# lbroseus/TALC

Hardware: AMD Instinct MI355X
Metric: corrected long-read bases/sec (whole node); k-mer-probe HBM GB/s (higher is better)
Workload: dtype u8

## Files before the change

talc_amd/csrc/pure_capi.cpp:

```cpp
#include <algorithm>
#include <cstdint>
#include <vector>

#include "talc_pure.h"
#include "talc_wfa.h"

using namespace talc;

extern "C" {

int pure_is_expected_by_model(double alpha, uint32_t nextc, uint32_t cc, int classe_unexpected) {
  return is_expected_by_model(alpha, nextc, cc, classe_unexpected != 0) ? 1 : 0;
}
int pure_is_expected_by_last_node(double alpha, uint32_t nextc, uint32_t cc) {
  return is_expected_by_last_node(alpha, nextc, cc) ? 1 : 0;
}
int pure_tag_next_nodes(double alpha, double err, uint32_t minc, const uint32_t* cnt4, const uint32_t* jc4, uint32_t count,
                        int complex, int32_t* tags4, double* dist4) {
  int t[4];
  double d[4];
  int n = tag_next_nodes(alpha, err, minc, cnt4, jc4, count, complex != 0, t, d);
  for (int i = 0; i < 4; ++i) { tags4[i] = t[i]; dist4[i] = d[i]; }
  return n;
}
// ... 16 lines not shown
void pure_gnu_heapsort_pairs(int32_t* keys, int32_t* payloads, int n) {
  std::vector<KP> v(n);
  for (int i = 0; i < n; ++i) v[i] = KP{keys[i], payloads[i]};
  gs_heapsort(v.data(), 0, n, KPLess());
  for (int i = 0; i < n; ++i) { keys[i] = v[i].key; payloads[i] = v[i].payload; }
}
void pure_std_heapsort_pairs(int32_t* keys, int32_t* payloads, int n) {
  std::vector<KP> v(n);
  for (int i = 0; i < n; ++i) v[i] = KP{keys[i], payloads[i]};
  std::partial_sort(v.begin(), v.end(), v.end(), KPLess());
  for (int i = 0; i < n; ++i) { keys[i] = v[i].key; payloads[i] = v[i].payload; }
}

int pure_gardening(uint32_t maxb, int n, const double* scores, const double* dists, uint32_t* kept, int32_t* isComplex) {
  std::vector<ValIdx> wv(n + 1);
  std::vector<Rank4> r1(n + 1), r2(n + 1);
  bool cx = false;
  int nk = gardening(maxb, n, scores, dists, wv.data(), r1.data(), r2.data(), kept, &cx);
  *isComplex = cx ? 1 : 0;
  return nk;
}

void pure_sort_anchors(double cc, uint32_t* pos, uint32_t* count, int n) {
  std::vector<AnchorRec> a(n);
  for (int i = 0; i < n; ++i) a[i] = AnchorRec{0, 0, pos[i], count[i]};
  gnu_sort(a.data(), n, LessAnchor{cc});
  for (int i = 0; i < n; ++i) { pos[i] = a[i].pos; count[i] = a[i].count; }
}

void pure_wfa_xdrop(const uint8_t* q, int qlen, const uint8_t* d, int dlen, int x, int32_t* out4) {
  const WfaResult r = wfa_xdrop_scalar(q, qlen, d, dlen, x);
  out4[0] = r.moved; out4[1] = r.extCols; out4[2] = r.extRows; out4[3] = r.score;
}
}
```

talc_amd/csrc/talc_kernels_search.h:

```cpp
#pragma once
#include "talc_common.h"
#include "talc_kernels_probe.h"
#include "talc_pure.h"
#include "talc_wave.h"

namespace talc {

#define TCAP 288
#define NBUF (2 * TCAP)
#ifndef LDS_DP_CAP
#define LDS_DP_CAP 320
#endif
#ifndef HOT
#define HOT 8
#endif
#ifndef AIMS_LDS
#define AIMS_LDS 16
#endif

enum : uint32_t {
  OVF_ANCHORS = 1, OVF_FULLPATHS = 2, OVF_FULLPOOL = 4, OVF_TRAILS = 8, OVF_SEQ = 16, OVF_OUT = 32, OVF_WEAKPOOL = 64,
  OVF_REGIONS = 128, OVF_DP = 256
};

// ... 504 lines not shown
struct TrailSet {
  uint64_t* kmer; uint64_t* nmask; double* dist; uint32_t* cnt; int32_t* score; uint32_t* fail; int32_t* lanc;
  int32_t* ranc; uint32_t* buf;
};
TALC_D TrailSet make_set(uint8_t* meta) {
  TrailSet s;
  s.kmer = (uint64_t*)(meta + TrailSetLayout::kmer); s.nmask = (uint64_t*)(meta + TrailSetLayout::nmask);
  s.dist = (double*)(meta + TrailSetLayout::dist); s.cnt = (uint32_t*)(meta + TrailSetLayout::cnt);
  s.score = (int32_t*)(meta + TrailSetLayout::score); s.fail = (uint32_t*)(meta + TrailSetLayout::fail);
  s.lanc = (int32_t*)(meta + TrailSetLayout::lanc); s.ranc = (int32_t*)(meta + TrailSetLayout::ranc);
  s.buf = (uint32_t*)(meta + TrailSetLayout::buf);
  return s;
}

struct TrailRec { uint64_t kmer, nmask; double dist; uint32_t cnt; int32_t score; uint32_t fail; int32_t lanc, ranc; uint32_t buf; };

#define LSYNC() do { __builtin_amdgcn_fence(__ATOMIC_ACQ_REL, "wavefront"); __builtin_amdgcn_wave_barrier(); } while (0)

__shared__ TrailRec g_hot[2 * HOT];
__shared__ uint64_t g_aimK[AIMS_LDS], g_aimN[AIMS_LDS];
__shared__ uint32_t g_aimPos[AIMS_LDS];
#define BLOOM_WORDS 128
__shared__ unsigned long long g_bloom[BLOOM_WORDS];
__shared__ __attribute__((aligned(16))) int g_dp[3 * LDS_DP_CAP];

struct EdgeCand {
  bool have; double score; double dist; double idscore; uint32_t len; uint32_t lanc, ranc;
};

enum { PF_PROBE = 0, PF_CHILD, PF_AIMS, PF_CYCLE, PF_FFWD, PF_SCOREBR, PF_GARDEN, PF_EVALFULL, PF_XDROP, PF_EXTNW,
       PF_EDGEMISC, PF_ANCHORS, PF_ASSEMBLE, PF_STEPB, PF_STEPE, PF_SRCHB, PF_SRCHE, PF_PROLOG, PF_INITTR, PF_TOTAL, PF_NCALLS, PF_NSTEPS,
       PF_FFLOAD, PF_FFREC, PF_FFFLUSH, PF_FFENTRY, PF_NRECS, PF_RD0, PF_RD1, PF_RD2, PF_RD3, PF_RD4, PF_RD5, PF_RDMAX,
       PF_XSTAGE, PF_XLEV, PF_XSEL, PF_REFB, PF_RESULT, PF_CYQ, PF_CYX, PF_CYHIT, PF_CYFILL,
       PF_SB11, PF_SB12, PF_SB21, PF_SB10, PF_SBOTHER, PF_SEGEN, PF_XCALLS, PF_XNLEV, PF_FSFORK, PF_FSDEAD, PF_FSFILT, PF_FSLIM, PF_FK1, PF_FK2, PF_FKBAIL, PF_FORK, PF_ANCCALLS, PF_ANCITER, PF_TPUB, PF_TOWN, PF_TSTOLEN, PF_TWAIT, PF_TRUN, PF_EA0, PF_EA1, PF_EA2, PF_EA3, PF_EA4, PF_EASUM3, PF_EASUM4, PF_RANCH, PF_RANCHMAX, PF_RBR, PF_RBRMAX, PF_N };
#define TALC_PF_NAMES {"probe", "child", "aims", "cycle", "ffwd", "scorebr", "garden", "evalfull", "xdrop", "extnw", "edgemisc", \
                       "anchors", "assemble", "stepb*", "stepe*", "srchb*", "srche*", "prolog", "inittr", "total", "#ffcalls", "#ffsteps", \
                       "ff.load", "ff.record", "ff.flush", "ff.entry", "#ffrecords", "#reads<0.25ms", "#reads<1ms", "#reads<4ms", \
                       "#reads<16ms", "#reads<64ms", "#reads>=64ms", "maxread(10ns)", "x.stage", "x.levels", "x.select", "b.ref", "b.result", \
                       "#cyc.query", "#cyc.exact", "#cyc.found", "cyc.fill%sum", \
                       "#stepb 1->1", "#stepb 1->2", "#stepb 2->1", "#stepb 1->0", "#stepb other", "#stepe generic", "#xdrop calls", "#xdrop levels", \
                       "#ffstop fork", "#ffstop deadend", "#ffstop filter", "#ffstop limit/other", "#forkstep 1 child", "#forkstep fork+deadend", "#forkstep bailed", "forkstep", "#anchor lists", "#anchor level tests", \
                       "#edges published", "#anchors by owner", "#anchors by others", "t.owner waits", "t.run by others", \
                       "#edge anchors<1ms", "#edge anchors<4ms", "#edge anchors<16ms", "#edge anchors<64ms", "#edge anchors>=64ms", "ticks anchors 16-64ms", "ticks anchors>=64ms", "(per read) anchors", "(per read) longest anchor", "(per read) bridge attempts", "(per read) longest bridge attempt"}

struct Wv {
  DevParams P; TableView T; SearchLimits C;
  const uint8_t* read; uint32_t L, n; const uint2* cov; double lambda;
  TrailSet G[2];
  int ia;
  uint8_t* seqPool;
  uint32_t nBuf;
  unsigned long long freeMask[NBUF / 64];
  uint8_t *ref, *fullPool, *edgeLong, *edgeShort, *edgeTmp, *weak;
  AnchorRec *ancL, *ancR; uint32_t* ancPos;
  FullMeta* fullMeta;
  int *dpG;
  double* gScores; double* gDists; ValIdx* gVal; Rank4* gRank; uint32_t* gKept;
  uint32_t *regS, *regE, *wOff, *wLen;
  int location, dirRight;
  uint32_t Ls, Le, Rs, Re;
  uint32_t weakLen;
  bool complexRegion;
  bool ffPopped;
  int nAncL, nAncR;
  uint32_t refLen;
  int nFull; uint32_t fullUsed;
  EdgeCand best2[2];
  int nEdges;
  unsigned long long cells, steps;
  uint32_t overflow;
  const TraceBuf* tracep;
  bool tracing, traceSteps;
  unsigned long long* wideBloom;
  int* rowPool;
  uint32_t searchNo;
  uint32_t rowStride, rowAvail;
// ... 552 lines not shown
      wave_xdrop<int*, false>(q, qlen, d, dlen, 0, -1, -1, xdrop, buf, extCols, extRows, ncells);
  }
  X.cells += ncells;
  return ((unsigned long long)(uint32_t)uni(extRows) << 32) | (uint32_t)uni(extCols);
}

struct SeedExt { int lenRefExt, lenHistExt, posOnRef, score; bool stop; int extRef, extCand; bool fallback; };

template <int MODE, bool LEAF = false>
TALC_D SeedExt seed_and_extension_body(const uint8_t* ref, int refLen, const uint8_t* cand, int candLen, int xdrop,
                                       bool withScore, uint32_t keepKey = 0) {
  PROF_DECL;
  refLen = uni(refLen); candLen = uni(candLen); xdrop = uni(xdrop); ref = uni_ptr(ref); cand = uni_ptr(cand);
  const int K = (int)X.P.K;
  const int S = X.dirRight ? K - 1 : K;
  SeedExt r;
  r.stop = false; r.score = 0; r.fallback = false;
  const bool state = !(refLen < candLen);
  const uint8_t* seq1 = state ? ref : cand; const int len1 = state ? refLen : candLen;
  const uint8_t* seq2 = state ? cand : ref; const int len2 = state ? candLen : refLen;
  int extCols = 0, extRows = 0, extScore = 0, rc = 0;
  unsigned long long ncells = 0;
  const int qlen = len2 - S, dlen = len1 - S;
  if (qlen > 0 && dlen > 0) {
    PROF_BEGIN();
#ifdef TALC_PROF
    if (lane_id() == 0) g_prof[PF_XCALLS] += 1;
#endif
    constexpr int STAGE = 3 * LDS_DP_CAP * 4;
    uint8_t TALC_AS3* stage = (uint8_t TALC_AS3*)g_dp;
    const int ndiagonals = min(max(xdrop, 0), qlen) + min(max(xdrop, 0), dlen) + 1;
    if (MODE == 2) {
      int* mem = X.dpG + 2ull * X.C.dpCap + 256;
      WfaPhase ph{-1, 31, mem, mem + 512};
      rc = wave_xdrop_wfa<1>(seq2 + S, qlen, seq1 + S, dlen, xdrop, stage, STAGE, extCols, extRows, extScore, ncells, &ph);
      if (rc == 2) {
        ph.fromLevel = 31; ph.toLevel = 63;
        rc = wave_xdrop_wfa<2>(seq2 + S, qlen, seq1 + S, dlen, xdrop, stage, STAGE, extCols, extRows, extScore, ncells, &ph);
        if (rc == 2) {
          ph.fromLevel = 63; ph.toLevel = 127;
          rc = wave_xdrop_wfa<4>(seq2 + S, qlen, seq1 + S, dlen, xdrop, stage, STAGE, extCols, extRows, extScore, ncells, &ph);
          if (rc == 2) {
            ph.fromLevel = 127; ph.toLevel = (ndiagonals <= 511) ? -1 : 255;
            rc = wave_xdrop_wfa<8>(seq2 + S, qlen, seq1 + S, dlen, xdrop, stage, STAGE, extCols, extRows, extScore, ncells, &ph);
            if (rc == 2) {
              ph.fromLevel = 255; ph.toLevel = -1;
              rc = wave_xdrop_wfa<16>(seq2 + S, qlen, seq1 + S, dlen, xdrop, stage, STAGE, extCols, extRows, extScore, ncells, &ph);
            }
          }
        }
      }
    }
    else if (MODE == 0 && ndiagonals <= 63) rc = wave_xdrop_wfa<1>(seq2 + S, qlen, seq1 + S, dlen, xdrop, stage, STAGE, extCols, extRows, extScore, ncells, nullptr, state ? keepKey : 0u);
    else if (MODE == 1 && ndiagonals <= 255) {
      int* mem = X.dpG + 2ull * X.C.dpCap + 256;
      WfaPhase ph{-1, 31, mem, mem + 512};
      rc = wave_xdrop_wfa<1>(seq2 + S, qlen, seq1 + S, dlen, xdrop, stage, STAGE, extCols, extRows, extScore, ncells, &ph, state ? keepKey : 0u);
      if (rc == 2) {
        ph.fromLevel = 31; ph.toLevel = (ndiagonals <= 127) ? -1 : 63;
        rc = wave_xdrop_wfa<2>(seq2 + S, qlen, seq1 + S, dlen, xdrop, stage, STAGE, extCols, extRows, extScore, ncells, &ph);
        if (rc == 2) {
          ph.fromLevel = 63; ph.toLevel = -1;
          rc = wave_xdrop_wfa<4>(seq2 + S, qlen, seq1 + S, dlen, xdrop, stage, STAGE, extCols, extRows, extScore, ncells, &ph);
        }
      }
    }
    else rc = -1;
    if (LEAF && rc < 0) { r.fallback = true; return r; }
    if (rc < 0) {
      rc = -1;
      const unsigned long long packed = xdrop_sweep(seq2 + S, qlen, seq1 + S, dlen, xdrop);
      extCols = (int)(uint32_t)packed; extRows = (int)(uint32_t)(packed >> 32);
    }
    PROF_END(PF_XDROP);
    X.cells += ncells;
  }
  const int ext1 = extRows, ext2 = extCols;
  r.extRef = state ? ext1 : ext2;
  r.extCand = state ? ext2 : ext1;
  r.lenRefExt = S + r.extRef;
  r.lenHistExt = S + r.extCand;
  r.posOnRef = X.dirRight ? (S + r.extRef) : (refLen - K - r.extRef);
  if (max(r.lenRefExt, r.lenHistExt) >= K) {
    if (withScore) {
      bool sameAnchor = LEAF && rc == 1;
      if (LEAF && !sameAnchor) { r.fallback = true; return r; }
      if (!LEAF && rc == 1) {
        const int l = lane_id();
        sameAnchor = ballot64(l < S && ((gcu8)ref)[l < S ? l : 0] != ((gcu8)cand)[l < S ? l : 0]) == 0ull;
      }
// ... 1927 lines not shown
  X.ia = 0;
  X.seqPool = slot + C.o_seqPool;
  X.refBuf = slot + C.o_ref; X.ref = X.refBuf; X.ancL = (AnchorRec*)(slot + C.o_ancL); X.ancR = (AnchorRec*)(slot + C.o_ancR);
  X.ancPos = (uint32_t*)(slot + C.o_ancPos);
  X.fullMeta = (FullMeta*)(slot + C.o_fullMeta); X.fullPool = slot + C.o_fullPoolB;
  X.edgeLong = slot + C.o_edgeLong; X.edgeShort = slot + C.o_edgeShort; X.edgeTmp = slot + C.o_edgeTmp;
  X.dpG = (int*)(slot + C.o_dp);
  X.wideBloom = (unsigned long long*)(slot + C.o_wideBloom); X.wideMask = 0;
  X.rowPool = (int*)(slot + C.o_rowPool); X.rowStride = 0; X.rowAvail = 0;
  X.launchStamp = launchStamp;
  if (E.boxes != nullptr && E.autoSwitch != nullptr && *E.autoSwitch == 0u) E.boxes = nullptr;
  X.boxes = E.boxes; X.avail = E.avail; X.qwords = queue; X.boxSeqCap = E.seqCap; X.boxBytes = (uint32_t)edge_box_bytes(E.seqCap);
  X.nSlots = gridDim.x; X.mySlot = blockIdx.x; X.nWork = n_work; X.taskMinWeak = E.minWeak; X.nanSeen = 0u; X.taskTest = E.test;
  X.taskHeavy = E.heavy; X.heavyUpTo = (E.heavyRounds >= 0xFFFFu) ? 0xFFFFFFFFu : E.heavyRounds * gridDim.x;
  X.qi = 0; X.holding = 0u; X.stealSeq = 0u; X.moreCells = 0; X.moreSteps = 0;
  const uint32_t lingerMod = max(E.lingerMod, 1u);
  X.searchNo = 16u;
  {
    uint8_t* g = slot + C.o_gard;
    X.gScores = (double*)g; g += 8ull * (TCAP + 64);
    X.gDists = (double*)g; g += 8ull * (TCAP + 64);
    X.gVal = (ValIdx*)g; g += 16ull * (TCAP + 64);
    X.gRank = (Rank4*)g; g += 32ull * (TCAP + 64);
    X.gKept = (uint32_t*)g;
  }
  X.regS = (uint32_t*)(slot + C.o_regS); X.regE = (uint32_t*)(slot + C.o_regE); X.regH = (uint32_t*)(slot + C.o_regH);
  X.wOff = (uint32_t*)(slot + C.o_wOff); X.wLen = (uint32_t*)(slot + C.o_wLen);
  X.weak = slot + C.o_weak;
  if (l == 0) *(TraceBuf*)(slot + C.o_trace) = trace;
  X.tracep = (const TraceBuf*)(slot + C.o_trace);
  unsigned long long totCells = 0, totSteps = 0;
  PROF_DECL2;
#ifdef TALC_PROF
  if (l == 0) { for (int i = 0; i < PF_N; ++i) g_prof[i] = 0; for (int i = 0; i < 4; ++i) g_wprof[i] = 0; }
  const unsigned long long _pf_k0 = __builtin_amdgcn_s_memtime();
  const unsigned long long _pf_r0 = __builtin_amdgcn_s_memrealtime();
  unsigned long long _pf_rd0 = 0, _pf_lastStart = 0, _pf_loopEnd = 0, _pf_idle = 0;
  uint32_t _pf_prevQi = 0, _pf_prevR = 0;
#endif

  while (true) {
    WSYNC();
#ifdef TALC_PROF
    if (l == 0 && _pf_rd0) {
      const unsigned long long dt = __builtin_amdgcn_s_memrealtime() - _pf_rd0;
      const int bk = dt < 25000ull ? 0 : dt < 100000ull ? 1 : dt < 400000ull ? 2 : dt < 1600000ull ? 3 : dt < 6400000ull ? 4 : 5;
      g_prof[PF_RD0 + bk] += 1;
      if (dt > g_prof[PF_RDMAX]) g_prof[PF_RDMAX] = (uint32_t)dt;
      state[_pf_prevR].pfTicks = (uint32_t)dt;
      _pf_lastStart = _pf_rd0; _pf_rd0 = 0;
    }
#endif
    if (X.boxes != nullptr) edge_between_reads();
    if (l == 0) s_next = atomicAdd(queue, 1u);
    WSYNC();
    const uint32_t qi = s_next;
    if (qi >= n_work) break;
    X.qi = qi;
#ifdef TALC_PROF
    _pf_rd0 = __builtin_amdgcn_s_memrealtime();
#endif
    PROF_BEGIN2();
    const uint32_t r = order[qi];
#ifdef TALC_PROF
    if (l == 0) state[r].pfStart = (uint32_t)_pf_rd0;
#endif
#ifdef TALC_PROF
// ... 134 lines not shown
        if (X.wLen[i] != 0xFFFFFFFFu) { copy_bytes(out + pos, X.weak + X.wOff[i], X.wLen[i], false); pos += X.wLen[i]; }
        else if (X.regS[i + 1] > e + K) { const uint32_t wl = X.regS[i + 1] - (e + K); copy_bytes(out + pos, X.read + e + K, wl, false); pos += wl; }
      }
    }
    if (tailPresent) {
      if (tailCorr) { copy_bytes(out + pos, X.weak + tailOff, tailCLen, false); pos += tailCLen; }
      else { copy_bytes(out + pos, X.read + (L - tailLen), tailLen, false); pos += tailLen; }
    }
    {
      unsigned long long part = 0;
      for (uint32_t i = l; i < R; i += 64) part += (unsigned long long)X.regE[i] - X.regS[i] + 1;
      const uint32_t span = (uint32_t)wave_sum_u64(part);
      if (l == 0) { state[r].outLen = pos; state[r].inSpan = span; }
    }
    PROF_END2(PF_ASSEMBLE);
  }
#ifdef TALC_PROF
  _pf_loopEnd = __builtin_amdgcn_s_memrealtime();
  if (l == 0) atomicMin((unsigned long long*)&counters[124], _pf_loopEnd);
#endif
  if (X.boxes != nullptr && blockIdx.x % lingerMod == 0u) {
#ifdef TALC_PROF
    _pf_idle =
#endif
    edge_linger(n_work);
  }
  totCells += X.moreCells; totSteps += X.moreSteps;
  if (l == 0) {
    if (totSteps) atomicAdd((unsigned long long*)&counters[0], totSteps);
    if (totCells) atomicAdd((unsigned long long*)&counters[1], totCells);
#ifdef TALC_PROF
    g_prof[PF_TOTAL] = (uint32_t)(__builtin_amdgcn_s_memtime() - _pf_k0);
    g_prof[PF_XSTAGE] = g_wprof[0]; g_prof[PF_XLEV] = g_wprof[1]; g_prof[PF_XSEL] = g_wprof[2]; g_prof[PF_XNLEV] = g_wprof[3];
    {
      const unsigned long long r1 = __builtin_amdgcn_s_memrealtime();
      atomicAdd((unsigned long long*)&counters[125], r1 - _pf_r0 - _pf_idle);
      atomicMin((unsigned long long*)&counters[126], _pf_r0);
      atomicMax((unsigned long long*)&counters[127], r1);
      if (_pf_rd0) state[_pf_prevR].pfTicks = (uint32_t)(r1 - _pf_rd0);
      if (blockIdx.x < 8192u) {
        counters[128 + 2 * blockIdx.x] = ((unsigned long long)_pf_prevQi << 32) | _pf_prevR;
        counters[129 + 2 * blockIdx.x] = ((_pf_lastStart & 0xFFFFFFFFull) << 32) | (_pf_loopEnd & 0xFFFFFFFFull);
      }
      static_assert(2 + PF_N <= 124, "the profile categories run into the utilisation counters");
    }
    for (int i = 0; i < PF_N; ++i) {
      if (i == PF_RDMAX) atomicMax((unsigned long long*)&counters[2 + i], (unsigned long long)g_prof[i]);
      else atomicAdd((unsigned long long*)&counters[2 + i], (unsigned long long)g_prof[i]);
    }
#endif
  }
}

TALC_D uint32_t order_bucket(const ReadState& st, uint32_t gapScale) {
  if (st.status != TALC_READ_CORRECTED || st.overflow) return 1023u;
  const unsigned long long key = (unsigned long long)st.costEst + (((unsigned long long)st.costGap * (gapScale - 256u)) >> 8);
  const uint32_t c = (uint32_t)min(key, 0xFFFFFFFFull) | 1u;
  const int e = 31 - __builtin_clz(c);
  const uint32_t m = (e >= 5) ? ((c >> (e - 5)) & 31u) : ((c << (5 - e)) & 31u);
  return 1022u - min(1022u, (uint32_t)e * 32u + m);
}
__global__ void __launch_bounds__(64) k_order_scale(uint32_t* __restrict__ batchStats) {
  const int l = lane_id();
  const unsigned long long fork = wave_sum_u64(batchStats[2 * l]), solid = wave_sum_u64(batchStats[2 * l + 1]);
  uint32_t scale = 256u;
  if (solid > 0) {
// ... 160 lines not shown
```

talc_amd/csrc/talc_wave.h:

```cpp
#pragma once
#include <limits.h>

#include "talc_common.h"

namespace talc {

#define WSYNC() __syncthreads()

TALC_D int lane_id() { return (int)__builtin_amdgcn_mbcnt_hi(~0u, __builtin_amdgcn_mbcnt_lo(~0u, 0u)); }
TALC_D int lane_id_here() { int l = lane_id(); asm volatile("" : "+v"(l)); return l; }
#define TALC_WAVE_REDUCE(v, OP, IDENT)                                                                   \
  do {                                                                                                   \
    v = OP(v, __builtin_amdgcn_update_dpp(IDENT, v, 0x111, 0xF, 0xF, false));                            \
    v = OP(v, __builtin_amdgcn_update_dpp(IDENT, v, 0x112, 0xF, 0xF, false));                            \
    v = OP(v, __builtin_amdgcn_update_dpp(IDENT, v, 0x114, 0xF, 0xF, false));                            \
    v = OP(v, __builtin_amdgcn_update_dpp(IDENT, v, 0x118, 0xF, 0xF, false));                            \
    v = OP(v, __builtin_amdgcn_update_dpp(IDENT, v, 0x142, 0xA, 0xF, false));                            \
    v = OP(v, __builtin_amdgcn_update_dpp(IDENT, v, 0x143, 0xC, 0xF, false));                            \
  } while (0)
TALC_D int wave_max_i32(int v) {
  TALC_WAVE_REDUCE(v, max, INT_MIN);
  return __builtin_amdgcn_readlane(v, 63);
}
TALC_D int talc_or_i32(int a, int b) { return a | b; }
// ... 516 lines not shown
    int mn, mx;
    minmaxS(A, false, mn, mx);
    const int lo = max(1 + mn, A + 3 - rows), hi = min(2 + mx, cols);
    early = lo >= hi;
  }
  if (!early) return firstMax(A);
  int maxColA = 1;
  if (A >= 2) {
    int mn1, mx1, mn2, mx2;
    minmaxS(A - 1, true, mn1, mx1);
    minmaxS(A - 2, false, mn2, mx2);
    const int cm = max(mx1, mx2);
    maxColA = (cm == INT_MIN) ? cols : min(2 + cm, cols);
  }
  const int c2 = maxColA - 1;
  if (kept(A, c2)) { take(A, c2); return 1; }
  if (A >= 2 && kept(A, c2 - 1)) { take(A, c2 - 1); return 1; }
  return firstMax(A - 1);
}

TALC_D void stage_copy(uint8_t TALC_AS3* dst, gcu8 src, int n) {
  const int l = lane_id_here();
  typedef uint64_t __attribute__((aligned(1))) u64u;
  const int nw = n >> 3;
  for (int w = l; w < nw; w += 64) ((uint64_t TALC_AS3*)dst)[w] = *(const u64u TALC_AS1*)(src + 8 * w);
  const int t = (nw << 3) + l;
  if (t < n) dst[t] = src[t];
}

struct WfaPhase {
  int fromLevel;
  int toLevel;
  int* memF; int* memE;
};

#ifdef TALC_PROF
__shared__ uint32_t g_wprof[4];
#define WPROF_T() __builtin_amdgcn_s_memtime()
#define WPROF_ADD(i, t0) (g_wprof[i] += (uint32_t)(__builtin_amdgcn_s_memtime() - (t0)))
#else
#define WPROF_T() 0ull
#define WPROF_ADD(i, t0) ((void)(t0))
#endif

struct WfaKeep { uint32_t owner; int level; int qlenAt; int pad_; uint16_t F[64]; uint8_t E[64]; };
__shared__ WfaKeep g_keep;

template <int NR>
TALC_D int wave_xdrop_wfa(const uint8_t* __restrict__ querySeg_, int qlen, const uint8_t* __restrict__ dbSeg_, int dlen, int x,
                          uint8_t TALC_AS3* stage, int stageCap, int& extCols, int& extRows, int& extScore,
                          unsigned long long& cells, const WfaPhase* ph = nullptr, uint32_t keepKey_ = 0) {
  gcu8 querySeg = (gcu8)uni_ptr(querySeg_); gcu8 dbSeg = (gcu8)uni_ptr(dbSeg_);
  const int l = lane_id();
  qlen = uni(qlen); dlen = uni(dlen); x = uni(x);
  extCols = extRows = extScore = 0;
  if (qlen <= 0 || dlen <= 0) return 0;
  const int NEG = -(1 << 29);
  const int X = min(max(x, 0), 1 << 20);
  const int fromLevel = ph ? ph->fromLevel : -1, toLevel = ph ? ph->toLevel : -1;
  const int Xm = (toLevel >= 0) ? min(X, toLevel) : X;
  const int kmin = -min(Xm, dlen), kmax = min(Xm, qlen);
  const int nd = kmax - kmin + 1;
  if (nd > 64 * NR - 1) return -1;
  const int qS = min(qlen, dlen + X), dS = min(dlen, qlen + X);
  const int qpad = (qS + 16) & ~7;
  if (qpad + dS + 16 > stageCap) return -1;
  const unsigned long long _t0 = WPROF_T();
  if (fromLevel < 0) {
    stage_copy(stage, querySeg, qS);
    stage_copy(stage + qpad, dbSeg, dS);
    if (l == 0) { stage[qS] = 0xF0; stage[qpad + dS] = 0xF1; }
  }
  WSYNC();
  WPROF_ADD(0, _t0);
  const unsigned long long _t1 = WPROF_T();
  const int bmax = x >= 2 ? x - 1 : (x == 1 ? 1 : 0);
  const int corner = qlen + dlen;
  int F[NR], E[NR], amax[NR], forb[NR];
#pragma unroll
  for (int s = 0; s < NR; ++s) {
    const int j = 64 * s + l, k = kmin + j, ak = k < 0 ? -k : k;
    amax[s] = (j < nd) ? min(2 * qlen - k, 2 * dlen + k) : NEG;
    forb[s] = (ak == bmax + 1) ? ak : -1;
    F[s] = NEG; E[s] = 0;
  }
  auto extend = [&](int (&a)[NR], bool (&act)[NR]) { wfa_extend<NR>(stage, qpad, kmin, a, act); };
  bool cornerHit = false;
  int cornerE = 0;
  int eStart = 1;
  const uint32_t keepKey = (NR == 1 && fromLevel < 0) ? (uint32_t)uni((int)keepKey_) : 0u;
  bool tracking = keepKey != 0u;
  const int kOfLane = kmin + l;
  const int aq = 2 * qlen - kOfLane;
  bool resumed = false;
  if (NR == 1 && keepKey != 0u) {
    const int lv = uni(g_keep.level), qat = uni(g_keep.qlenAt);
// ... 11 lines not shown
    if (level >= 1 && level <= 31) {
      if (l < nd) { g_keep.F[(kOfLane + 32) & 63] = (uint16_t)(F[0] >= 0 ? F[0] : 0xFFFF); g_keep.E[(kOfLane + 32) & 63] = (uint8_t)E[0]; }
      if (l == 0) { g_keep.owner = keepKey; g_keep.level = level; g_keep.qlenAt = qlen; }
    }
  };
  if (resumed) {
  } else
  if (fromLevel >= 0) {
#pragma unroll
    for (int s = 0; s < NR; ++s) {
      const int j = 64 * s + l, k = kmin + j, ak = k < 0 ? -k : k;
      const bool in = (j < nd) & (ak <= fromLevel);
      F[s] = in ? ph->memF[in ? k + 256 : 256] : NEG;
      E[s] = in ? ph->memE[in ? k + 256 : 256] : 0;
    }
    eStart = fromLevel + 1;
  } else {
    int a0[NR]; bool act0[NR];
    const int j0 = -kmin;
#pragma unroll
    for (int s = 0; s < NR; ++s) { a0[s] = 0; act0[s] = (64 * s + l == j0) && x >= 0; }
    extend(a0, act0);
#pragma unroll
    for (int s = 0; s < NR; ++s) if (64 * s + l == j0) F[s] = a0[s];
    unsigned long long hit = 0;
#pragma unroll
    for (int s = 0; s < NR; ++s) hit |= ballot64(F[s] == corner);
    cornerHit = hit != 0ull;
    if (tracking && ballot64(F[0] == aq) != 0ull) tracking = false;
  }
  const int eEnd = (toLevel >= 0) ? min(x, toLevel) : x;
  unsigned long long work = 0;
  const int kc = qlen - dlen;
  const bool cornerInBand = (kc >= kmin) & (kc <= kmax);
  int eLast = eStart - 1;
  for (int e = eStart; e <= eEnd && !cornerHit; ++e) {
    if (NR == 1 && tracking && e == x) { keep_level(e - 1); tracking = false; }
    const bool forbLevel = (e == bmax + 1);
    int rotR[NR], rotL[NR];
#pragma unroll
    for (int s = 0; s < NR; ++s) { rotR[s] = lane_ror1(F[s]); rotL[s] = lane_rol1(F[s]); }
    const int sLo = max(0, -e - kmin) >> 6, sHi = min(nd - 1, e - kmin) >> 6;
    int b[NR]; bool act[NR];
#pragma unroll
    for (int s = 0; s < NR; ++s) {
      b[s] = NEG; act[s] = false;
      if (NR == 1 || (s >= sLo && s <= sHi)) {
        const int fl = (NR > 1 && l == 0) ? rotR[(s + NR - 1) % NR] : rotR[s];
        const int fr = (NR > 1 && l == 63) ? rotL[(s + 1) % NR] : rotL[s];
        int v2 = fl + 1; v2 = (v2 <= amax[s]) ? v2 : NEG;
        int v3 = fr + 1; v3 = (v3 <= amax[s]) ? v3 : NEG;
        int v = max(max(v2, v3), min(F[s] + 2, amax[s]));
        if (forbLevel) v = (v == forb[s]) ? NEG : v;
        b[s] = v;
        act[s] = (v > F[s]) & (v >= 0);
      }
    }
    bool moved[NR];
#pragma unroll
    for (int s = 0; s < NR; ++s) moved[s] = act[s];
    extend(b, act);
    if (NR == 1 && tracking && ballot64(b[0] == aq) != 0ull) {
      keep_level(e - 1);
      tracking = false;
    }
    unsigned long long hit = 0;
#pragma unroll
    for (int s = 0; s < NR; ++s) {
      if (moved[s]) { F[s] = b[s]; E[s] = e; }
      if (cornerInBand) hit |= ballot64(F[s] == corner);
    }
    if (hit != 0ull) { cornerHit = true; cornerE = e; }
    eLast = e;
  }
  if (NR == 1 && tracking && !cornerHit && eLast < x) keep_level(eLast);
  if (eLast >= eStart) {
    const int eh = min(eLast, (nd - 1) / 2);
    const int lo = max(eh, eStart - 1);
    if (eh >= eStart) work += (unsigned long long)((eh - eStart + 1) * (eh + eStart + 1));
    if (eLast > lo) work += (unsigned long long)((eLast - lo) * nd);
  }
  cells += work;
  WPROF_ADD(1, _t1);
#ifdef TALC_PROF
  if (eLast >= eStart) g_wprof[3] += (uint32_t)(eLast - eStart + 1);
#endif
  const unsigned long long _t2 = WPROF_T();
  if (cornerHit) { extCols = qlen; extRows = dlen; extScore = -cornerE; return 1; }
  if (toLevel >= 0 && toLevel < x) {
#pragma unroll
    for (int s = 0; s < NR; ++s) {
      const int j = 64 * s + l, k = kmin + j, ak = k < 0 ? -k : k;
      if ((j < nd) & (ak <= toLevel)) { ph->memF[k + 256] = F[s]; ph->memE[k + 256] = E[s]; }
    }
    WSYNC();
    return 2;
  }
  const int rsel = wfa_select<NR>(F, E, kmin, kmax, qlen, dlen, extCols, extRows, extScore);
  WPROF_ADD(2, _t2);
  return rsel;
}

template <int NR>
TALC_D int wave_xdrop_wfa_multi(const uint8_t* __restrict__ querySeg_, int qlen, const uint8_t* __restrict__ dbSeg_, int dlen, int xHi,
                                uint8_t TALC_AS3* stage, int stageCap, int* resCols, int* resRows, int* resScore,
                                unsigned long long& cells) {
  gcu8 querySeg = (gcu8)uni_ptr(querySeg_); gcu8 dbSeg = (gcu8)uni_ptr(dbSeg_);
  const int l = lane_id();
  qlen = uni(qlen); dlen = uni(dlen); xHi = uni(xHi);
  if (qlen <= 0 || dlen <= 0 || xHi < 0) return -1;
  const int NEG = -(1 << 29);
  const int X = min(xHi, 1 << 20);
  const int kmin = -min(X, dlen), kmax = min(X, qlen);
  const int nd = kmax - kmin + 1;
  if (nd > 64 * NR - 1) return -1;
  const int qS = min(qlen, dlen + X), dS = min(dlen, qlen + X);
  const int qpad = (qS + 16) & ~7;
  if (qpad + dS + 16 > stageCap) return -1;
  stage_copy(stage, querySeg, qS);
  stage_copy(stage + qpad, dbSeg, dS);
  if (l == 0) { stage[qS] = 0xF0; stage[qpad + dS] = 0xF1; }
  WSYNC();
  const int corner = qlen + dlen;
  int F[NR], E[NR], amax[NR], ak[NR];
#pragma unroll
  for (int s = 0; s < NR; ++s) {
    const int j = 64 * s + l, k = kmin + j;
    ak[s] = k < 0 ? -k : k;
    amax[s] = (j < nd) ? min(2 * qlen - k, 2 * dlen + k) : NEG;
    F[s] = NEG; E[s] = 0;
  }
// ... 315 lines not shown
```

talc_amd/csrc/talc_wfa.h:

```cpp
#pragma once
#include <climits>
#include <cstdint>
#include <vector>

namespace talc {

struct WfaResult { int moved; int extCols; int extRows; int score; };

inline WfaResult wfa_xdrop_scalar(const uint8_t* q, int qlen, const uint8_t* d, int dlen, int x) {
  WfaResult res = {0, 0, 0, 0};
  if (qlen == 0 || dlen == 0) return res;
  const int NEG = -(1 << 29);
  const int bmax = x >= 2 ? x - 1 : (x == 1 ? 1 : 0);
  const int X = x < 0 ? 0 : x;
  const int kmin = -(X < dlen ? X : dlen), kmax = (X < qlen ? X : qlen);
  const int nd = kmax - kmin + 1;
  std::vector<int> F(nd + 2, NEG), G(nd + 2, NEG), E(nd + 2, 0), amin(nd + 2), amax(nd + 2);
  auto idx = [&](int k) { return k - kmin + 1; };
  for (int k = kmin; k <= kmax; ++k) {
    const int ak = k < 0 ? -k : k;
    amin[idx(k)] = ak + (ak > bmax ? 2 : 0);
    const int a1 = 2 * qlen - k, a2 = 2 * dlen + k;
    amax[idx(k)] = a1 < a2 ? a1 : a2;
  }
  auto extend = [&](int a, int k) {
    int c = (a + k) / 2, r = (a - k) / 2;
    while (c < qlen && r < dlen && q[c] == d[r]) { ++c; ++r; }
    return c + r;
  };
  const int corner = qlen + dlen, kc = qlen - dlen;
  F[idx(0)] = x >= 0 ? extend(0, 0) : 0;
  bool cornerHit = (kc >= kmin && kc <= kmax && F[idx(kc)] == corner);
  int cornerE = 0;
  for (int e = 1; e <= x && !cornerHit; ++e) {
    for (int k = kmin; k <= kmax; ++k) {
      const int i = idx(k);
      const int fm = F[i], fl = F[i - 1], fr = F[i + 1];
      int best = NEG;
      const int v[3] = {fm + 2, fl + 1, fr + 1};
      for (int t = 0; t < 3; ++t)
        if (v[t] >= amin[i] && v[t] <= amax[i] && v[t] > best) best = v[t];
      int nv = fm;
      if (best > fm) { nv = extend(best, k); E[i] = e; }
      G[i] = nv;
    }
    F.swap(G);
    if (kc >= kmin && kc <= kmax && F[idx(kc)] == corner) { cornerHit = true; cornerE = e; }
  }
  if (cornerHit) { res.moved = 1; res.extCols = qlen; res.extRows = dlen; res.score = -cornerE; return res; }
  int A = 0;
  for (int k = kmin; k <= kmax; ++k) if (F[idx(k)] > A) A = F[idx(k)];
  const int cols = qlen + 1, rows = dlen + 1;
  auto minmaxS = [&](int a, bool dropTopBorder, int& mn, int& mx) {
    mn = INT_MAX; mx = INT_MIN;
    if (a < 0) return;
    for (int k = kmin; k <= kmax; ++k) {
      if (((k - a) & 1) || F[idx(k)] < a) continue;
      const int c = (a + k) / 2;
      if (dropTopBorder && c == a) continue;
      if (c < mn) mn = c;
      if (c > mx) mx = c;
    }
  };
  auto kept = [&](int a, int c) {
    const int k = 2 * c - a;
    return c >= 0 && a - c >= 0 && k >= kmin && k <= kmax && F[idx(k)] >= a;
  };
  auto firstMax = [&](int a) {
    int bestE = INT_MAX, bestK = 0;
    for (int k = kmin; k <= kmax; ++k) {
      if (((k - a) & 1) || F[idx(k)] != a) continue;
      if (E[idx(k)] < bestE) { bestE = E[idx(k)]; bestK = k; }
    }
    if (bestE == INT_MAX) return;
    res.moved = 1; res.extCols = (a + bestK) / 2; res.extRows = (a - bestK) / 2; res.score = -bestE;
  };
  bool early = false;
  if (A + 1 >= 2) {
    int mn, mx; minmaxS(A, false, mn, mx);
    const int a = A + 1;
// ... 27 lines not shown
```

Before: 4.654 billion.

## Run X-drop WFA past level 31 in a sliding one-wave diagonal window

Adds a windowed mode to the single-register WFA kernel. Once three adjacent diagonals have reached the query end, diagonals above them are treated as dead, so the 64-lane band is shifted downward by bpermute instead of escalating to the multi-register (NR=2/4) phases. This targets the cost of wider-band phases for long X-drop extensions. It adds a ballot and permute per shifted level, a bail-out path when the window cannot shift, a scalar reference that implements the same pruning, and an exhaustive equivalence checker. Correctness depends on the pruning rule exactly matching the full-band result.

Result: faster. 4.716 billion, median of 6 (+1.3%).

```diff
diff --git a/talc_amd/csrc/pure_capi.cpp b/talc_amd/csrc/pure_capi.cpp
--- a/talc_amd/csrc/pure_capi.cpp
+++ b/talc_amd/csrc/pure_capi.cpp
@@ -72,4 +72,30 @@
   const WfaResult r = wfa_xdrop_scalar(q, qlen, d, dlen, x);
   out4[0] = r.moved; out4[1] = r.extCols; out4[2] = r.extRows; out4[3] = r.score;
 }
+void pure_wfa_xdrop_full(const uint8_t* q, int qlen, const uint8_t* d, int dlen, int x, int32_t* out4) {
+  const WfaResult r = wfa_xdrop_scalar(q, qlen, d, dlen, x, false);
+  out4[0] = r.moved; out4[1] = r.extCols; out4[2] = r.extRows; out4[3] = r.score;
 }
+int pure_wfa_window_exhaustive(int maxQ, int maxD, int xLo, int xHi, int64_t* runs, int32_t* first5) {
+  int bad = 0;
+  int64_t n = 0;
+  uint8_t q[32], d[32];
+  for (int ql = 1; ql <= maxQ; ++ql)
+    for (uint32_t qb = 0; qb < (1u << ql); ++qb)
+      for (int dl = 1; dl <= maxD; ++dl)
+        for (uint32_t db = 0; db < (1u << dl); ++db) {
+          for (int i = 0; i < ql; ++i) q[i] = (uint8_t)((qb >> i) & 1u);
+          for (int i = 0; i < dl; ++i) d[i] = (uint8_t)((db >> i) & 1u);
+          for (int x = xLo; x <= xHi; ++x) {
+            const WfaResult a = wfa_xdrop_scalar(q, ql, d, dl, x, true), b = wfa_xdrop_scalar(q, ql, d, dl, x, false);
+            ++n;
+            if (a.moved != b.moved || a.extCols != b.extCols || a.extRows != b.extRows || a.score != b.score) {
+              if (bad == 0) { first5[0] = (int32_t)qb; first5[1] = ql; first5[2] = (int32_t)db; first5[3] = dl; first5[4] = x; }
+              ++bad;
+            }
+          }
+        }
+  *runs = n;
+  return bad;
+}
+}
diff --git a/talc_amd/csrc/talc_kernels_search.h b/talc_amd/csrc/talc_kernels_search.h
--- a/talc_amd/csrc/talc_kernels_search.h
+++ b/talc_amd/csrc/talc_kernels_search.h
@@ -560,7 +560,7 @@
        PF_EDGEMISC, PF_ANCHORS, PF_ASSEMBLE, PF_STEPB, PF_STEPE, PF_SRCHB, PF_SRCHE, PF_PROLOG, PF_INITTR, PF_TOTAL, PF_NCALLS, PF_NSTEPS,
        PF_FFLOAD, PF_FFREC, PF_FFFLUSH, PF_FFENTRY, PF_NRECS, PF_RD0, PF_RD1, PF_RD2, PF_RD3, PF_RD4, PF_RD5, PF_RDMAX,
        PF_XSTAGE, PF_XLEV, PF_XSEL, PF_REFB, PF_RESULT, PF_CYQ, PF_CYX, PF_CYHIT, PF_CYFILL,
-       PF_SB11, PF_SB12, PF_SB21, PF_SB10, PF_SBOTHER, PF_SEGEN, PF_XCALLS, PF_XNLEV, PF_FSFORK, PF_FSDEAD, PF_FSFILT, PF_FSLIM, PF_FK1, PF_FK2, PF_FKBAIL, PF_FORK, PF_ANCCALLS, PF_ANCITER, PF_TPUB, PF_TOWN, PF_TSTOLEN, PF_TWAIT, PF_TRUN, PF_EA0, PF_EA1, PF_EA2, PF_EA3, PF_EA4, PF_EASUM3, PF_EASUM4, PF_RANCH, PF_RANCHMAX, PF_RBR, PF_RBRMAX, PF_N };
+       PF_SB11, PF_SB12, PF_SB21, PF_SB10, PF_SBOTHER, PF_SEGEN, PF_XCALLS, PF_XNLEV, PF_FSFORK, PF_FSDEAD, PF_FSFILT, PF_FSLIM, PF_FK1, PF_FK2, PF_FKBAIL, PF_FORK, PF_ANCCALLS, PF_ANCITER, PF_TPUB, PF_TOWN, PF_TSTOLEN, PF_TWAIT, PF_TRUN, PF_EA0, PF_EA1, PF_EA2, PF_EA3, PF_EA4, PF_EASUM3, PF_EASUM4, PF_RANCH, PF_RANCHMAX, PF_RBR, PF_RBRMAX, PF_XNLEVW, PF_XNLEVWIN, PF_N };
 #define TALC_PF_NAMES {"probe", "child", "aims", "cycle", "ffwd", "scorebr", "garden", "evalfull", "xdrop", "extnw", "edgemisc", \
                        "anchors", "assemble", "stepb*", "stepe*", "srchb*", "srche*", "prolog", "inittr", "total", "#ffcalls", "#ffsteps", \
                        "ff.load", "ff.record", "ff.flush", "ff.entry", "#ffrecords", "#reads<0.25ms", "#reads<1ms", "#reads<4ms", \
@@ -569,7 +569,8 @@
                        "#stepb 1->1", "#stepb 1->2", "#stepb 2->1", "#stepb 1->0", "#stepb other", "#stepe generic", "#xdrop calls", "#xdrop levels", \
                        "#ffstop fork", "#ffstop deadend", "#ffstop filter", "#ffstop limit/other", "#forkstep 1 child", "#forkstep fork+deadend", "#forkstep bailed", "forkstep", "#anchor lists", "#anchor level tests", \
                        "#edges published", "#anchors by owner", "#anchors by others", "t.owner waits", "t.run by others", \
-                       "#edge anchors<1ms", "#edge anchors<4ms", "#edge anchors<16ms", "#edge anchors<64ms", "#edge anchors>=64ms", "ticks anchors 16-64ms", "ticks anchors>=64ms", "(per read) anchors", "(per read) longest anchor", "(per read) bridge attempts", "(per read) longest bridge attempt"}
+                       "#edge anchors<1ms", "#edge anchors<4ms", "#edge anchors<16ms", "#edge anchors<64ms", "#edge anchors>=64ms", "ticks anchors 16-64ms", "ticks anchors>=64ms", "(per read) anchors", "(per read) longest anchor", "(per read) bridge attempts", "(per read) longest bridge attempt", \
+                       "#xdrop levels >=2 per lane", "#xdrop levels windowed"}
 
 struct Wv {
   DevParams P; TableView T; SearchLimits C;
@@ -1188,8 +1189,12 @@
     const int ndiagonals = min(max(xdrop, 0), qlen) + min(max(xdrop, 0), dlen) + 1;
     if (MODE == 2) {
       int* mem = X.dpG + 2ull * X.C.dpCap + 256;
-      WfaPhase ph{-1, 31, mem, mem + 512};
-      rc = wave_xdrop_wfa<1>(seq2 + S, qlen, seq1 + S, dlen, xdrop, stage, STAGE, extCols, extRows, extScore, ncells, &ph);
+      WfaPhase ph{-1, 31, mem, mem + 512, -1};
+      rc = wave_xdrop_wfa<1, true>(seq2 + S, qlen, seq1 + S, dlen, xdrop, stage, STAGE, extCols, extRows, extScore, ncells, &ph);
+      if (ph.winLast > 31) {
+        const int X = max(xdrop, 0);
+        ncells += wfa_phases_cells(ph.winLast, qlen, dlen, X, {63, 127, 255, INT_MAX}, {63, 127, ndiagonals <= 511 ? X : 255, X});
+      }
       if (rc == 2) {
         ph.fromLevel = 31; ph.toLevel = 63;
         rc = wave_xdrop_wfa<2>(seq2 + S, qlen, seq1 + S, dlen, xdrop, stage, STAGE, extCols, extRows, extScore, ncells, &ph);
@@ -1210,8 +1215,12 @@
     else if (MODE == 0 && ndiagonals <= 63) rc = wave_xdrop_wfa<1>(seq2 + S, qlen, seq1 + S, dlen, xdrop, stage, STAGE, extCols, extRows, extScore, ncells, nullptr, state ? keepKey : 0u);
     else if (MODE == 1 && ndiagonals <= 255) {
       int* mem = X.dpG + 2ull * X.C.dpCap + 256;
-      WfaPhase ph{-1, 31, mem, mem + 512};
-      rc = wave_xdrop_wfa<1>(seq2 + S, qlen, seq1 + S, dlen, xdrop, stage, STAGE, extCols, extRows, extScore, ncells, &ph, state ? keepKey : 0u);
+      WfaPhase ph{-1, 31, mem, mem + 512, -1};
+      rc = wave_xdrop_wfa<1, true>(seq2 + S, qlen, seq1 + S, dlen, xdrop, stage, STAGE, extCols, extRows, extScore, ncells, &ph, state ? keepKey : 0u);
+      if (ph.winLast > 31) {
+        const int X = max(xdrop, 0);
+        ncells += wfa_phases_cells(ph.winLast, qlen, dlen, X, {63, INT_MAX, INT_MAX, INT_MAX}, {ndiagonals <= 127 ? X : 63, X, X, X});
+      }
       if (rc == 2) {
         ph.fromLevel = 31; ph.toLevel = (ndiagonals <= 127) ? -1 : 63;
         rc = wave_xdrop_wfa<2>(seq2 + S, qlen, seq1 + S, dlen, xdrop, stage, STAGE, extCols, extRows, extScore, ncells, &ph);
@@ -3205,7 +3214,7 @@
   unsigned long long totCells = 0, totSteps = 0;
   PROF_DECL2;
 #ifdef TALC_PROF
-  if (l == 0) { for (int i = 0; i < PF_N; ++i) g_prof[i] = 0; for (int i = 0; i < 4; ++i) g_wprof[i] = 0; }
+  if (l == 0) { for (int i = 0; i < PF_N; ++i) g_prof[i] = 0; for (int i = 0; i < 6; ++i) g_wprof[i] = 0; }
   const unsigned long long _pf_k0 = __builtin_amdgcn_s_memtime();
   const unsigned long long _pf_r0 = __builtin_amdgcn_s_memrealtime();
   unsigned long long _pf_rd0 = 0, _pf_lastStart = 0, _pf_loopEnd = 0, _pf_idle = 0;
@@ -3406,6 +3415,7 @@
 #ifdef TALC_PROF
     g_prof[PF_TOTAL] = (uint32_t)(__builtin_amdgcn_s_memtime() - _pf_k0);
     g_prof[PF_XSTAGE] = g_wprof[0]; g_prof[PF_XLEV] = g_wprof[1]; g_prof[PF_XSEL] = g_wprof[2]; g_prof[PF_XNLEV] = g_wprof[3];
+    g_prof[PF_XNLEVW] = g_wprof[4]; g_prof[PF_XNLEVWIN] = g_wprof[5];
     {
       const unsigned long long r1 = __builtin_amdgcn_s_memrealtime();
       atomicAdd((unsigned long long*)&counters[125], r1 - _pf_r0 - _pf_idle);
diff --git a/talc_amd/csrc/talc_wave.h b/talc_amd/csrc/talc_wave.h
--- a/talc_amd/csrc/talc_wave.h
+++ b/talc_amd/csrc/talc_wave.h
@@ -572,10 +572,34 @@
   int fromLevel;
   int toLevel;
   int* memF; int* memE;
+  int winLast;
 };
 
+TALC_D unsigned long long wfa_levels_cells(int eStart, int eLast, int nd) {
+  unsigned long long work = 0;
+  if (eLast >= eStart) {
+    const int eh = min(eLast, (nd - 1) / 2);
+    const int lo = max(eh, eStart - 1);
+    if (eh >= eStart) work += (unsigned long long)((eh - eStart + 1) * (eh + eStart + 1));
+    if (eLast > lo) work += (unsigned long long)((eLast - lo) * nd);
+  }
+  return work;
+}
+
+TALC_D unsigned long long wfa_phases_cells(int last, int qlen, int dlen, int X, const int (&to)[4], const int (&y)[4]) {
+  unsigned long long w = 0;
+  int from = 31;
+  for (int i = 0; i < 4 && from < last; ++i) {
+    const int Y = min(X, y[i]), hi = min(last, to[i]);
+    w += wfa_levels_cells(from + 1, hi, min(Y, dlen) + min(Y, qlen) + 1);
+    from = hi;
+  }
+  return w;
+}
+
+
 #ifdef TALC_PROF
-__shared__ uint32_t g_wprof[4];
+__shared__ uint32_t g_wprof[6];
 #define WPROF_T() __builtin_amdgcn_s_memtime()
 #define WPROF_ADD(i, t0) (g_wprof[i] += (uint32_t)(__builtin_amdgcn_s_memtime() - (t0)))
 #else
@@ -586,10 +610,10 @@
 struct WfaKeep { uint32_t owner; int level; int qlenAt; int pad_; uint16_t F[64]; uint8_t E[64]; };
 __shared__ WfaKeep g_keep;
 
-template <int NR>
+template <int NR, bool WIN = false>
 TALC_D int wave_xdrop_wfa(const uint8_t* __restrict__ querySeg_, int qlen, const uint8_t* __restrict__ dbSeg_, int dlen, int x,
                           uint8_t TALC_AS3* stage, int stageCap, int& extCols, int& extRows, int& extScore,
-                          unsigned long long& cells, const WfaPhase* ph = nullptr, uint32_t keepKey_ = 0) {
+                          unsigned long long& cells, WfaPhase* ph = nullptr, uint32_t keepKey_ = 0) {
   gcu8 querySeg = (gcu8)uni_ptr(querySeg_); gcu8 dbSeg = (gcu8)uni_ptr(dbSeg_);
   const int l = lane_id();
   qlen = uni(qlen); dlen = uni(dlen); x = uni(x);
@@ -599,9 +623,12 @@
   const int X = min(max(x, 0), 1 << 20);
   const int fromLevel = ph ? ph->fromLevel : -1, toLevel = ph ? ph->toLevel : -1;
   const int Xm = (toLevel >= 0) ? min(X, toLevel) : X;
-  const int kmin = -min(Xm, dlen), kmax = min(Xm, qlen);
+  int kmin = -min(Xm, dlen);
+  const int kmax = min(Xm, qlen);
   const int nd = kmax - kmin + 1;
   if (nd > 64 * NR - 1) return -1;
+  static_assert(!WIN || NR == 1, "the live window is a one-diagonal-per-lane phase");
+  if (WIN) ph->winLast = -1;
   const int qS = min(qlen, dlen + X), dS = min(dlen, qlen + X);
   const int qpad = (qS + 16) & ~7;
   if (qpad + dS + 16 > stageCap) return -1;
@@ -679,9 +706,33 @@
   const int eEnd = (toLevel >= 0) ? min(x, toLevel) : x;
   unsigned long long work = 0;
   const int kc = qlen - dlen;
-  const bool cornerInBand = (kc >= kmin) & (kc <= kmax);
+  bool cornerInBand = (kc >= kmin) & (kc <= kmax);
   int eLast = eStart - 1;
-  for (int e = eStart; e <= eEnd && !cornerHit; ++e) {
+  const bool mayWin = WIN && toLevel >= 0 && toLevel < x;
+  const int kLoB = -min(X, dlen), kHiB = min(X, qlen);
+  bool winLost = false;
+  for (int e = eStart; e <= (mayWin ? x : eEnd) && !cornerHit; ++e) {
+    const bool winEnter = mayWin && e == toLevel + 1;
+    const bool winShift = mayWin && e > toLevel && -e < kmin && kmin > kLoB;
+    if (winEnter || winShift) {
+      const unsigned long long cl = ballot64(F[0] == 2 * qlen - (kmin + l));
+      const unsigned long long c3 = cl & (cl >> 1) & (cl >> 2);
+      if (winEnter && (c3 == 0ull || tracking)) break;
+      if (winShift) {
+        const int top = (int)__builtin_ctzll(c3) + 2;
+        const int sh = min(62 - top, kmin - kLoB);
+        if (sh < 1) { winLost = true; break; }
+        const int f = __builtin_amdgcn_ds_bpermute(((l - sh) & 63) << 2, F[0]);
+        const int ev = __builtin_amdgcn_ds_bpermute(((l - sh) & 63) << 2, E[0]);
+        const bool in = (l >= sh) & (l - sh <= top);
+        F[0] = in ? f : NEG; E[0] = in ? ev : 0;
+        kmin -= sh;
+        const int k = kmin + l, ak = k < 0 ? -k : k;
+        amax[0] = ((l < 63) & (k >= kLoB) & (k <= kHiB)) ? min(2 * qlen - k, 2 * dlen + k) : NEG;
+        forb[0] = (ak == bmax + 1) ? ak : -1;
+        cornerInBand = (kc >= kmin) & (kc <= min(kHiB, kmin + 62));
+      }
+    }
     if (NR == 1 && tracking && e == x) { keep_level(e - 1); tracking = false; }
     const bool forbLevel = (e == bmax + 1);
     int rotR[NR], rotL[NR];
@@ -721,20 +772,21 @@
     eLast = e;
   }
   if (NR == 1 && tracking && !cornerHit && eLast < x) keep_level(eLast);
-  if (eLast >= eStart) {
-    const int eh = min(eLast, (nd - 1) / 2);
-    const int lo = max(eh, eStart - 1);
-    if (eh >= eStart) work += (unsigned long long)((eh - eStart + 1) * (eh + eStart + 1));
-    if (eLast > lo) work += (unsigned long long)((eLast - lo) * nd);
-  }
+  work += wfa_levels_cells(eStart, (WIN && eLast > toLevel && toLevel >= 0) ? toLevel : eLast, nd);
   cells += work;
   WPROF_ADD(1, _t1);
 #ifdef TALC_PROF
-  if (eLast >= eStart) g_wprof[3] += (uint32_t)(eLast - eStart + 1);
+  if (eLast >= eStart) {
+    g_wprof[3] += (uint32_t)(eLast - eStart + 1);
+    if (NR > 1) g_wprof[4] += (uint32_t)(eLast - eStart + 1);
+    if (WIN && toLevel >= 0 && eLast > toLevel) g_wprof[5] += (uint32_t)(eLast - toLevel);
+  }
 #endif
   const unsigned long long _t2 = WPROF_T();
+  if (WIN && winLost) return -1;
+  if (WIN && toLevel >= 0 && eLast > toLevel) ph->winLast = eLast;
   if (cornerHit) { extCols = qlen; extRows = dlen; extScore = -cornerE; return 1; }
-  if (toLevel >= 0 && toLevel < x) {
+  if (toLevel >= 0 && toLevel < x && !(WIN && eLast > toLevel)) {
 #pragma unroll
     for (int s = 0; s < NR; ++s) {
       const int j = 64 * s + l, k = kmin + j, ak = k < 0 ? -k : k;
@@ -743,7 +795,8 @@
     WSYNC();
     return 2;
   }
-  const int rsel = wfa_select<NR>(F, E, kmin, kmax, qlen, dlen, extCols, extRows, extScore);
+  const int kmaxSel = (WIN && eLast > toLevel && toLevel >= 0) ? min(kHiB, kmin + 62) : kmax;
+  const int rsel = wfa_select<NR>(F, E, kmin, kmaxSel, qlen, dlen, extCols, extRows, extScore);
   WPROF_ADD(2, _t2);
   return rsel;
 }
diff --git a/talc_amd/csrc/talc_wfa.h b/talc_amd/csrc/talc_wfa.h
--- a/talc_amd/csrc/talc_wfa.h
+++ b/talc_amd/csrc/talc_wfa.h
@@ -7,7 +7,7 @@
 
 struct WfaResult { int moved; int extCols; int extRows; int score; };
 
-inline WfaResult wfa_xdrop_scalar(const uint8_t* q, int qlen, const uint8_t* d, int dlen, int x) {
+inline WfaResult wfa_xdrop_scalar(const uint8_t* q, int qlen, const uint8_t* d, int dlen, int x, bool window = true) {
   WfaResult res = {0, 0, 0, 0};
   if (qlen == 0 || dlen == 0) return res;
   const int NEG = -(1 << 29);
@@ -32,9 +32,11 @@
   F[idx(0)] = x >= 0 ? extend(0, 0) : 0;
   bool cornerHit = (kc >= kmin && kc <= kmax && F[idx(kc)] == corner);
   int cornerE = 0;
+  int top = kmax;
   for (int e = 1; e <= x && !cornerHit; ++e) {
     for (int k = kmin; k <= kmax; ++k) {
       const int i = idx(k);
+      if (k > top) { G[i] = NEG; continue; }
       const int fm = F[i], fl = F[i - 1], fr = F[i + 1];
       int best = NEG;
       const int v[3] = {fm + 2, fl + 1, fr + 1};
@@ -46,6 +48,15 @@
     }
     F.swap(G);
     if (kc >= kmin && kc <= kmax && F[idx(kc)] == corner) { cornerHit = true; cornerE = e; }
+    if (window) {
+      for (int k = kmin; k + 2 <= top; ++k) {
+        if (F[idx(k)] == 2 * qlen - k && F[idx(k + 1)] == 2 * qlen - k - 1 && F[idx(k + 2)] == 2 * qlen - k - 2) {
+          top = k + 2;
+          for (int j = top + 1; j <= kmax; ++j) F[idx(j)] = NEG;
+          break;
+        }
+      }
+    }
   }
   if (cornerHit) { res.moved = 1; res.extCols = qlen; res.extRows = dlen; res.score = -cornerE; return res; }
   int A = 0;
```
